# guisongchen/vo_slam_test

Measured on AMD Instinct MI355X. Metric: tracked frames/sec + local-BA LM-iters/sec (synthetic 640x480; value = tracked frames/sec: ORB extraction, frame post-processing, two guided searches with the culling / isInFrame steps between them and two pose-only solves per frame, one vo_tracker C call per batch), higher is better.
Workload: dtype u8; 1 GPU; tracked frame: ORB extract (640x480, 8-level pyramid, 1000 kpts) + undistort/depth/grid + searchByProjection vs last frame + solvePoseOnlySE3 + cullingOutliersBeforeLocalMap + isInFrame (refined pose) + searchByProjection vs local map + solvePoseOnlySE3; frames, depth and map resident in HBM; parallelism=frames sharded x1, no collective, batches_in_flight=2

## Files before the change

vo_slam_test_amd/csrc/orb.hip:

```cpp
#include "vo_common.h"

#include <cmath>
#include <mutex>
#include <vector>

namespace {

using namespace vo;

constexpr int kMaxLevels = 16;
constexpr int kEdge = 19;
constexpr int kBorder = kEdge - 3;
constexpr int kHalfPatch = 15;
constexpr int kTileP = 72;
constexpr int kFastCpw = 4;
constexpr int kMaxList = 1024;

__constant__ __attribute__((aligned(16))) uint32_t c_desc_tab[64][36];
const int8_t h_pattern[1024] = {
#include "orb_pattern.inc"
};

struct LevelGeom {
  int w, h, pitch;
// ... 346 lines not shown
        const lds_u8 *b = (const lds_u8 *)(uintptr_t)(unsigned)plist[i];
        pos = (int)(b - tile);
        const lds_u8 *c = b + sdelta + 2 * TP + 2;
        sc0 = c[TP + 1];
        const unsigned nb = max_u16(max_u16(max_u16(c[0], c[1]), max_u16(c[2], c[TP])),
                                    max_u16(max_u16(c[TP + 2], c[2 * TP]), max_u16(c[2 * TP + 1], c[2 * TP + 2])));
        keep = sc0 >= th && sc0 > (int)nb;
      }
      const unsigned long long mask = __builtin_amdgcn_ballot_w64(keep);
      const int off = kept + __builtin_amdgcn_mbcnt_hi((unsigned)(mask >> 32), __builtin_amdgcn_mbcnt_lo((unsigned)mask, 0u));
      if (keep && off < cap_cell) {
        const int y = pos / TP, x = pos - y * TP;
        slot[off] = (uint32_t)(x + 3 + xoff) | ((uint32_t)(y + 3 + yoff) << 12) | ((uint32_t)sc0 << 24);
      }
      kept += __popcll(mask);
    }
    return kept;
  };
  int running = 0;
  for (int round = 0; round < 2; round++) {
    const int th = round == 0 ? ini_th : min_th;
    const int np0 = walk(th, 0, ih);
    wave_sync();
    int np = np0;
    if (np <= list_cap - 64) {
      if (round == 1) {
        if (np > 64) np = refine_list(np, th, ring_k2);
        if (np > 64) np = refine_list(np, th, ring_k1);
        if (np > 64) np = refine_list(np, th, ring_k3);
      }
      score_list(np);
      wave_sync();
      running = nms_list(np, th, 0);
    } else {
      const int chunk_rows = max((list_cap - 64) / 64, 1) * ri;
      for (int r0 = 0; r0 < ih; r0 += chunk_rows) {
        const int n = walk(th, r0, min(r0 + chunk_rows, ih));
        wave_sync();
        score_list(n);
        wave_sync();
      }
      running = 0;
      for (int r0 = 0; r0 < ih; r0 += chunk_rows) {
        const int n = walk(th, r0, min(r0 + chunk_rows, ih));
        wave_sync();
        running = nms_list(n, th, running);
        wave_sync();
      }
    }
    if (running > 0) break;
    wave_sync();
  }
  if (lane == 0) *out_count = min(running, cap_cell);
}

template <int TP, bool BYTEWISE>
__attribute__((amdgpu_waves_per_eu(8, 8))) __global__ __launch_bounds__(256) void k_fast_cell(OrbDev P, FrameSrc src, uint32_t *cell_slots,
                                                   long long slots_frame_stride, int *cell_count,
                                                   int cells_per_frame, int tile_rows, int list_cap,
                                                   const int *__restrict__ cell_tab, int cell_begin, int cell_end) {
  extern __shared__ __attribute__((aligned(16))) uint8_t fast_lds[];
  const int lane = threadIdx.x & 63;
  const int wave = __builtin_amdgcn_readfirstlane((int)threadIdx.x >> 6);
  const int f = blockIdx.y;
  for (int cpw = 0; cpw < kFastCpw; cpw++) {
  const int cell = cell_begin + (blockIdx.x * 4 + wave) * kFastCpw + cpw;
  if (cell >= cell_end) return;
  if (cpw) wave_sync();
  const int tile_bytes = fast_align16(TP * tile_rows);
  lds_u8 *tile_raw = (lds_u8 *)fast_lds + wave * fast_cell_lds(TP, tile_rows, list_cap);
  lds_u16 *plist = (lds_u16 *)(tile_raw + 2 * tile_bytes);
  const int *cd = cell_tab + 16 * cell;
  const int l = cd[0], iniX = cd[1], iniY = cd[2], cw = cd[3], ch = cd[4], xoff = cd[5], yoff = cd[6];
  const int slot_off = cd[7], cap_cell = cd[8];
  int *out_count = cell_count + (long long)f * cells_per_frame + cell;
  const int iw = cw - 6, ih = ch - 6;
  if (iw <= 0 || ih <= 0) {
    if (lane == 0) *out_count = 0;
    continue;
  }
  int pitch;
  const uint8_t *img;
  if (l == 0) {
    pitch = src.img0_pitch;
    img = src.img0 + (long long)f * src.img0_frame_stride;
  } else {
    pitch = cd[9];
    img = src.pyr + (long long)f * src.pyr_frame_stride + (((long long)cd[11] << 32) | (unsigned)cd[10]);
  }
  const bool bytewise = BYTEWISE && l == 0;
  const int ox = bytewise ? 0 : (iniX & 3);
  lds_u8 *tile = tile_raw + ox;
  const uint8_t *g0 = img + (long long)iniY * pitch + (iniX - ox);
  if (!bytewise && TP == 48) {
    gmem_u8 *gb = (gmem_u8 *)g0;
#pragma unroll
    for (int k = 0; k < 3; k++) {
      const int idx = lane + 64 * k;
      const unsigned row = (unsigned)idx / 3u, chunk = (unsigned)idx - 3u * row;
      if (64 * k < 3 * ch && idx < 3 * ch)
        __builtin_amdgcn_global_load_lds(gb + (row * (unsigned)pitch + 16u * chunk), tile_raw + 1024 * k, 16, 0, 0);
    }
  } else if (!bytewise) {
    constexpr int LW = TP <= 64 ? 16 : 32, RG = 64 / LW, NB = 6;
    const int npr = (ox + cw + 3) >> 2;
    const int d = lane & (LW - 1), r = lane / LW;
    if (d < npr) {
      const unsigned goff = (unsigned)(r * pitch + 4 * d);
      lds_u8 *lt = tile_raw + r * TP + 4 * d;
      const int ng = (ch + RG - 1) / RG, last0 = max(ch - RG, 0);
      for (int gb = 0; gb < ng; gb += NB) {
        uint32_t v[NB];
        int row0[NB];
#pragma unroll
        for (int q = 0; q < NB; q++) {
          row0[q] = min(min(gb + q, ng - 1) * RG, last0);
          long long ro = (long long)row0[q] * pitch;
          asm("" : "+s"(ro));
          v[q] = *reinterpret_cast<const uint32_t *>(g0 + ro + goff);
        }
#pragma unroll
        for (int q = 0; q < NB; q++) {
          int lo = row0[q] * TP;
          asm("" : "+s"(lo));
          *(__attribute__((address_space(3))) uint32_t *)(lt + lo) = v[q];
        }
      }
    }
  } else {
    constexpr int NB = 8;
    for (int col = lane; col < cw; col += 64) {
      for (int rb = 0; rb < ch; rb += NB) {
        uint8_t v[NB];
        int row[NB];
#pragma unroll
        for (int q = 0; q < NB; q++) {
          row[q] = min(rb + q, ch - 1);
          v[q] = g0[(long long)row[q] * pitch + col];
        }
#pragma unroll
        for (int q = 0; q < NB; q++) tile_raw[row[q] * TP + col] = v[q];
      }
    }
  }
  for (int i = lane; i < tile_bytes / 16; i += 64)
    *(__attribute__((address_space(3))) u32x4_t *)(tile_raw + tile_bytes + 16 * i) = u32x4_t{0u, 0u, 0u, 0u};
  asm volatile("s_waitcnt vmcnt(0)" ::: "memory");
  wave_sync();
  fast_cell_body<TP>(tile, tile_bytes, plist, list_cap, iw, ih, P.ini_th, P.min_th,
                     cell_slots + (long long)f * slots_frame_stride + slot_off, cap_cell, xoff, yoff, out_count, lane);
  }
}

__device__ __forceinline__ int block_excl_scan(int v, int *wsum , int *total) {
  const int lane = threadIdx.x & 63, wave = threadIdx.x >> 6;
  int x = v;
#pragma unroll
  for (int o = 1; o < 64; o <<= 1) {
    int y = __shfl_up(x, o);
    if (lane >= o) x += y;
  }
  __syncthreads();
  if (lane == 63) wsum[wave] = x;
  __syncthreads();
  int base = 0, tot = 0;
  for (int w = 0; w < 4; w++) {
    if (w < wave) base += wsum[w];
    tot += wsum[w];
  }
  *total = tot;
  return base + x - v;
}

template <int CAP>
struct OctLds {
  unsigned short x0[2][CAP], y0[2][CAP], x1[2][CAP], y1[2][CAP];
  unsigned short cnt[2][CAP], seq[2][CAP];
  unsigned short prank[CAP];
  unsigned short order[CAP];
  unsigned short newpos_old[CAP];
  unsigned short newpos_child[CAP * 4];
  int ccount[CAP * 4];
  int cprefix[CAP];
  unsigned int best[CAP];
  int wsum[8];
  int s_m, s_cutoff, s_newsize, s_nexp, s_total;
};

__device__ __forceinline__ int quadrant_of(int kx, int ky, int x0, int y0, int x1, int y1) {
  const int midx = x0 + ((x1 - x0 + 1) >> 1);
  const int midy = y0 + ((y1 - y0 + 1) >> 1);
  return (kx < midx ? 0 : 1) + (ky < midy ? 0 : 2);
}

template <int CAP>
__attribute__((amdgpu_waves_per_eu(kOctWaves, kOctWaves))) __global__ __launch_bounds__(256) void k_octree(OrbDev P, const uint32_t *cell_slots,
                                                long long slots_frame_stride, const int *cell_count,
                                                int cells_per_frame, uint32_t *key_data,
                                                unsigned short *key_label, int keys_per_frame,
                                                int *cand_count, uint32_t *sel, int sel_per_frame,
                                                int *nk, int *err_flag) {
  __shared__ OctLds<CAP> S;
  const int tid = threadIdx.x;
  const int l = blockIdx.y, f = blockIdx.x;
  const LevelGeom &L = P.lv[l];
  uint32_t *kd = key_data + (long long)f * keys_per_frame + L.candBase;
  unsigned short *kl = key_label + (long long)f * keys_per_frame + L.candBase;
  const int *cc = cell_count + (long long)f * cells_per_frame + L.cellBase;
  const uint32_t *slots = cell_slots + (long long)f * slots_frame_stride + L.slotBase;
  const int N = L.quota;

  constexpr int KR = 8;
  uint32_t kreg[KR];
  int lreg[KR];
  int n = 0;
  bool inreg;
  if (L.nCells <= CAP * 4) {
    int *coff = S.ccount;
    for (int base = 0; base < L.nCells; base += 256) {
      const int c = base + tid;
      const int cnt = c < L.nCells ? cc[c] : 0;
      int tot;
      const int off = n + block_excl_scan(cnt, S.wsum, &tot);
      if (c < L.nCells) coff[c] = off;
      n += tot;
    }
    __syncthreads();
    const int ncand = min(n, L.candCap);
    inreg = ncand <= 256 * KR;
    auto slot_of = [&](int k) {
      int lo = 0, hi = L.nCells - 1;
      while (lo < hi) {
        const int mid = (lo + hi + 1) >> 1;
        if (coff[mid] <= k) lo = mid; else hi = mid - 1;
      }
      return (long long)lo * L.capCell + (k - coff[lo]);
    };
#pragma unroll
    for (int e = 0; e < KR; e++) {
      const int k = tid + 256 * e;
      kreg[e] = k < ncand ? slots[slot_of(k)] : 0u;
      lreg[e] = 0;
    }
#pragma unroll
    for (int e = 0; e < KR; e++) {
      const int k = tid + 256 * e;
      if (k < ncand) kd[k] = kreg[e];
    }
    for (int k = tid + 256 * KR; k < ncand; k += 256) kd[k] = slots[slot_of(k)];
  } else {
    for (int base = 0; base < L.nCells; base += 256) {
      const int c = base + tid;
      const int cnt = c < L.nCells ? cc[c] : 0;
      int tot;
      const int off = n + block_excl_scan(cnt, S.wsum, &tot);
      for (int e0 = 0; e0 < cnt; e0 += 4) {
        uint32_t v[4];
#pragma unroll
        for (int u = 0; u < 4; u++) v[u] = slots[(long long)c * L.capCell + min(e0 + u, cnt - 1)];
#pragma unroll
        for (int u = 0; u < 4; u++)
          if (e0 + u < cnt && off + e0 + u < L.candCap) kd[off + e0 + u] = v[u];
      }
      n += tot;
    }
    __syncthreads();
    __threadfence_block();
    inreg = min(n, L.candCap) <= 256 * KR;
#pragma unroll
    for (int e = 0; e < KR; e++) {
      const int k = tid + 256 * e;
      kreg[e] = (inreg && k < min(n, L.candCap)) ? kd[k] : 0u;
      lreg[e] = 0;
    }
  }
  if (n > L.candCap) {
    if (tid == 0) atomicExch(err_flag, 1);
    n = L.candCap;
  }
  if (tid == 0) cand_count[f * P.nlevels + l] = n;
  __syncthreads();
  __threadfence_block();
  auto for_keys = [&](auto body) {
    if (inreg) {
#pragma unroll
      for (int e = 0; e < KR; e++) {
        const int k = tid + 256 * e;
        if (k < n) body(k, kreg[e], lreg[e]);
      }
    } else {
      for (int k = tid; k < n; k += 256) {
        int lab = kl[k];
        const int lab0 = lab;
        body(k, kd[k], lab);
        if (lab != lab0) kl[k] = (unsigned short)lab;
      }
    }
  };

  int cur = 0;
  const int nIni = L.nIni;
  const int H = L.maxBY - kBorder;
  for (int i = tid; i < CAP * 4; i += 256) S.ccount[i] = 0;
  __syncthreads();
  if (!inreg)
    for (int k = tid; k < n; k += 256) kl[k] = 0xffff;
  for_keys([&](int, uint32_t kv, int &lab) {
    const int kx = kv & 0xfff;
    int b = (int)((float)kx / L.hX);
    b = min(max(b, 0), nIni - 1);
    lab = b;
    atomicAdd(&S.ccount[b], 1);
  });
  __syncthreads();
  int size = 0;
  {
    if (tid == 0) {
      int s = 0;
      for (int i = 0; i < nIni && s < CAP; i++) {
        const int c = S.ccount[i];
        S.newpos_old[i] = 0xffff;
        if (c == 0) continue;
        S.x0[0][s] = (unsigned short)(int)(L.hX * (float)i);
        S.x1[0][s] = (unsigned short)(int)(L.hX * (float)(i + 1));
        S.y0[0][s] = 0;
        S.y1[0][s] = (unsigned short)H;
        S.cnt[0][s] = (unsigned short)min(c, 65535);
        S.seq[0][s] = (unsigned short)s;
        S.newpos_old[i] = (unsigned short)s;
        s++;
      }
      S.s_newsize = s;
    }
    __syncthreads();
    size = S.s_newsize;
    for_keys([&](int, uint32_t, int &lab) { lab = S.newpos_old[lab]; });
    __syncthreads();
  }

  bool careful = false;
  bool finish = (n == 0);
  int guard = 0;
  while (!finish && guard++ < 64) {
    const int prevSize = size;
    int myflag[4], myrank[4];
    int local = 0;
    for (int e = 0; e < 4; e++) {
      const int pos = tid * 4 + e;
      myflag[e] = (pos < size && S.cnt[cur][pos] > 1) ? 1 : 0;
      local += myflag[e];
    }
    int m;
    int ex = block_excl_scan(local, S.wsum, &m);
    for (int e = 0; e < 4; e++) {
      const int pos = tid * 4 + e;
      myrank[e] = ex;
      ex += myflag[e];
      if (pos < CAP) S.prank[pos] = myflag[e] ? (unsigned short)myrank[e] : 0xffff;
      if (myflag[e]) S.order[myrank[e]] = (unsigned short)pos;
    }
    __syncthreads();
    if (careful && m > 1) {
      for (int j = tid; j < m; j += 256) {
        const int p2 = S.order[j];
        S.cprefix[j] = (int)(((unsigned int)S.cnt[cur][p2] << 16) | S.seq[cur][p2]);
      }
      __syncthreads();
      int mypos[CAP / 256], myr[CAP / 256];
#pragma unroll
      for (int u = 0; u < CAP / 256; u++) {
        const int j = tid + 256 * u;
        mypos[u] = -1, myr[u] = 0;
        if (j >= m) continue;
        mypos[u] = S.order[j];
        const unsigned int mykey = (unsigned int)S.cprefix[j];
        int r = 0;
        for (int i = 0; i < m; i++) r += ((unsigned int)S.cprefix[i] > mykey) ? 1 : 0;
        myr[u] = r;
      }
      __syncthreads();
#pragma unroll
      for (int u = 0; u < CAP / 256; u++)
        if (mypos[u] >= 0) {
          S.prank[mypos[u]] = (unsigned short)myr[u];
          S.order[myr[u]] = (unsigned short)mypos[u];
        }
      __syncthreads();
    }
    for (int i = tid; i < m * 4; i += 256) S.ccount[i] = 0;
    __syncthreads();
    for_keys([&](int, uint32_t kv, int &lab) {
      const int pos = lab;
      const int r = S.prank[pos];
      if (r == 0xffff) return;
      const int q = quadrant_of(kv & 0xfff, (kv >> 12) & 0xfff, S.x0[cur][pos], S.y0[cur][pos], S.x1[cur][pos],
                                S.y1[cur][pos]);
      atomicAdd(&S.ccount[r * 4 + q], 1);
    });
    __syncthreads();
    {
      int run_c = 0;
      int cutoff = m - 1;
      bool found = false;
      for (int base = 0; base < m; base += 256) {
        const int r = base + tid;
        int c = 0;
        if (r < m)
          for (int q = 0; q < 4; q++) c += S.ccount[r * 4 + q] > 0;
        int tot;
        const int exs = block_excl_scan(c, S.wsum, &tot);
        const int inc = run_c + exs + c;
        if (r < m) S.cprefix[r] = inc;
        run_c += tot;
      }
      __syncthreads();
      if (careful) {
        if (tid == 0) S.s_cutoff = m - 1;
        __syncthreads();
        for (int r = tid; r < m; r += 256) {
          const int sz = prevSize + S.cprefix[r] - (r + 1);
          if (sz >= N) atomicMin(&S.s_cutoff, r);
        }
        __syncthreads();
        cutoff = S.s_cutoff;
        found = true;
      }
      (void)found;
      const int totalChildren = m > 0 ? S.cprefix[cutoff] : 0;
      const int nxt = cur ^ 1;
      if (tid == 0) S.s_nexp = 0;
      __syncthreads();
      int nexp_local = 0;
      for (int r = tid; r <= cutoff && r < m; r += 256) {
        const int pos = S.order[r];
        const int base_r = totalChildren - S.cprefix[r];
        const int px0 = S.x0[cur][pos], py0 = S.y0[cur][pos], px1 = S.x1[cur][pos], py1 = S.y1[cur][pos];
        const int midx = px0 + ((px1 - px0 + 1) >> 1), midy = py0 + ((py1 - py0 + 1) >> 1);
        int after = 0;
        for (int q = 3; q >= 0; q--) {
          const int c = S.ccount[r * 4 + q];
          if (c == 0) {
            S.newpos_child[r * 4 + q] = 0xffff;
            continue;
          }
          const int np = base_r + after;
          after++;
          S.newpos_child[r * 4 + q] = (unsigned short)np;
          S.x0[nxt][np] = (unsigned short)((q & 1) ? midx : px0);
          S.x1[nxt][np] = (unsigned short)((q & 1) ? px1 : midx);
          S.y0[nxt][np] = (unsigned short)((q & 2) ? midy : py0);
          S.y1[nxt][np] = (unsigned short)((q & 2) ? py1 : midy);
          S.cnt[nxt][np] = (unsigned short)min(c, 65535);
          S.seq[nxt][np] = (unsigned short)(r * 4 + q);
          nexp_local += c > 1;
        }
      }
      if (nexp_local) atomicAdd(&S.s_nexp, nexp_local);
      int keptlocal = 0, kf[4];
      for (int e = 0; e < 4; e++) {
        const int pos = tid * 4 + e;
        const int r = pos < size ? S.prank[pos] : 0xffff;
        kf[e] = (pos < size && (r == 0xffff || r > cutoff)) ? 1 : 0;
        keptlocal += kf[e];
      }
      int keptTotal;
      int kex = block_excl_scan(keptlocal, S.wsum, &keptTotal);
      for (int e = 0; e < 4; e++) {
        const int pos = tid * 4 + e;
        if (!kf[e]) {
          if (pos < CAP) S.newpos_old[pos] = 0xffff;
          continue;
        }
        const int np = totalChildren + kex;
        kex++;
        S.newpos_old[pos] = (unsigned short)np;
        if (np < CAP) {
          S.x0[nxt][np] = S.x0[cur][pos];
          S.x1[nxt][np] = S.x1[cur][pos];
          S.y0[nxt][np] = S.y0[cur][pos];
          S.y1[nxt][np] = S.y1[cur][pos];
          S.cnt[nxt][np] = S.cnt[cur][pos];
          S.seq[nxt][np] = S.seq[cur][pos];
        }
      }
      __syncthreads();
      const int newsize = totalChildren + keptTotal;
      for_keys([&](int, uint32_t kv, int &lab) {
        const int pos = lab;
        const int r = S.prank[pos];
        if (r != 0xffff && r <= cutoff) {
          const int q = quadrant_of(kv & 0xfff, (kv >> 12) & 0xfff, S.x0[cur][pos], S.y0[cur][pos],
                                    S.x1[cur][pos], S.y1[cur][pos]);
          lab = S.newpos_child[r * 4 + q];
        } else {
          lab = S.newpos_old[pos];
        }
      });
      __syncthreads();
      const int nToExpand = S.s_nexp;
      cur = nxt;
      size = newsize;
      if (size > CAP - 4) {
        if (tid == 0) atomicExch(err_flag, 2);
        finish = true;
      }
      if (size >= N || size == prevSize)
        finish = true;
      else if (!careful && size + nToExpand * 3 > N)
        careful = true;
    }
    __syncthreads();
  }

  for (int i = tid; i < CAP; i += 256) S.best[i] = 0;
  __syncthreads();
  for_keys([&](int k, uint32_t kv, int &lab) {
    const int pos = lab;
    if (pos >= CAP) return;
    const unsigned int v = ((kv >> 24) << 16) | (unsigned int)(65535 - k);
    atomicMax(&S.best[pos], v);
  });
  __syncthreads();
  uint32_t *out = sel + (long long)f * sel_per_frame + L.selBase;
  const int nout = min(size, L.capSel);
  for (int i = tid; i < nout; i += 256) out[i] = kd[65535 - (S.best[i] & 0xffff)];
  if (tid == 0) nk[f * P.nlevels + l] = (n == 0) ? 0 : nout;
}

__device__ __forceinline__ int reflect101(int i, int n) {
  if (n == 1) return 0;
  while (i < 0 || i >= n) i = i < 0 ? -i : 2 * n - 2 - i;
  return i;
}
__device__ __forceinline__ int reflect101_near(int i, int n) { return i < 0 ? -i : (i >= n ? 2 * n - 2 - i : i); }

__global__ __launch_bounds__(256) void k_blur(OrbDev P, FrameSrc src, unsigned level_mask) {
  __shared__ uint8_t t[22][72];
  __shared__ int hs[22][64];
  const int kq[7] = {18, 34, 49, 55, 49, 34, 18};
  const int tid = threadIdx.x, f = blockIdx.y;
  int tile = blockIdx.x;
  int l = 0;
  while (l + 1 < P.nlevels && tile >= P.lv[l + 1].tileBase) l++;
  const LevelGeom &L = P.lv[l];
  if (!((level_mask >> l) & 1u)) return;
  tile -= L.tileBase;
  const int ty = tile / L.tilesX, tx = tile - ty * L.tilesX;
  const int x0 = tx * 64, y0 = ty * 16;
  int pitch;
  const uint8_t *img = level_plane(P, src, l, f, pitch);
  for (int idx = tid; idx < 22 * 70; idx += 256) {
    const int r = idx / 70, c = idx - r * 70;
    const int sy = reflect101(y0 + r - 3, L.h), sx = reflect101(x0 + c - 3, L.w);
    t[r][c] = img[(long long)sy * pitch + sx];
  }
  __syncthreads();
  for (int idx = tid; idx < 22 * 64; idx += 256) {
    const int r = idx >> 6, c = idx & 63;
    int acc = 0;
#pragma unroll
    for (int i = 0; i < 7; i++) acc += kq[i] * t[r][c + i];
    hs[r][c] = acc;
  }
  __syncthreads();
  uint8_t *dst = src.blur + (long long)f * src.blur_frame_stride + L.blur_off;
  for (int idx = tid; idx < 16 * 64; idx += 256) {
    const int r = idx >> 6, c = idx & 63;
    if (x0 + c >= L.w || y0 + r >= L.h) continue;
    int acc = 0;
#pragma unroll
    for (int j = 0; j < 7; j++) acc += kq[j] * hs[r + j][c];
    const int v = (acc + (1 << 15)) >> 16;
    dst[blur_tiled_off(x0 + c, y0 + r, L.pitch)] = (uint8_t)min(v, 255);
  }
}

constexpr int kBlurB = 16;
constexpr int kBlurF = 64 / kBlurB;
constexpr int kBlurMinW = 24, kBlurMinH = 4;
constexpr int kBlurRows = 36;

__global__ __launch_bounds__(256) void k_blur_groups(FrameSrc src, int lv0_generic, const int *__restrict__ job_tab,
                                                     int n_jobs, int n_frames) {
  const int lane = threadIdx.x & 63;
  const int job = blockIdx.x * 4 + __builtin_amdgcn_readfirstlane((int)threadIdx.x >> 6);
  if (job >= n_jobs) return;
  const int *sd = job_tab + 16 * job;
  const int l = sd[0], cb = sd[1], sy = sd[2], Lh = sd[3], Lpitch = sd[4], ngroups = sd[5], w = sd[11];
  if (l == 0 && lv0_generic) return;
  const int f0 = blockIdx.y * kBlurF, fo = lane / kBlurB;
  const bool fvalid = f0 + fo < n_frames;
  const int fl = fvalid ? fo : 0;
  const int G = min(cb * kBlurB + (lane & (kBlurB - 1)), ngroups - 1), x = 4 * G;
  int pitch;
  const uint8_t *img;
  unsigned fsrc;
  if (l == 0) {
    pitch = src.img0_pitch;
    img = src.img0 + (long long)f0 * src.img0_frame_stride;
    fsrc = (unsigned)(fl * src.img0_frame_stride);
  } else {
    pitch = sd[8];
    img = src.pyr + (long long)f0 * src.pyr_frame_stride + (((long long)sd[10] << 32) | (unsigned)sd[9]);
    fsrc = (unsigned)(fl * src.pyr_frame_stride);
  }
  const int Gu = cb * kBlurB + (lane & (kBlurB - 1));
  const bool tile_ok = fvalid && 4 * (Gu & ~3) < Lpitch && (Gu & ~3) < ngroups;
  uint8_t *dst = src.blur + (long long)f0 * src.blur_frame_stride + (((long long)sd[7] << 32) | (unsigned)sd[6]) +
                 (long long)fl * src.blur_frame_stride + (Gu >> 2) * 128;
  __shared__ __attribute__((aligned(16))) unsigned tr_all[4][4][64];
  unsigned (*tr)[64] = tr_all[threadIdx.x >> 6];
  const unsigned vC = fsrc + (unsigned)x, vL = vC - (G > 0 ? 4u : 0u), vR = vC + (x + 4 < pitch ? 4u : 0u);
  const bool edge_job = cb == 0 || (cb + 1) * kBlurB * 4 + 4 > w;
  unsigned selC = 0x07060504u, selRA = 0x07060504u, selRB = 0u, selL = 0x03020100u;
  bool caseB = false, left = false;
  if (edge_job) {
    auto srck = [&](int k) {
      int i = x - 4 + k;
      if (i > w - 1) i = 2 * (w - 1) - i;
      return min(max(i - (x - 4), 0), 11);
    };
    selC = 0, selRA = 0, selRB = 0;
#pragma unroll
    for (int b = 0; b < 4; b++) {
      const int kc = srck(4 + b), kr = srck(8 + b);
      selC |= (unsigned)min(kc, 7) << (8 * b);
      selRA |= (unsigned)min(max(kr - 4, 0), 7) << (8 * b);
      selRB |= (unsigned)min(kr, 7) << (8 * b);
    }
    caseB = x + 4 > w - 1;
    left = G == 0;
    selL = 0x01020304u;
  }
  const int y0 = sy * kBlurRows, y1 = min(Lh, y0 + kBlurRows);
  const unsigned K0 = 18u | (34u << 8) | (49u << 16) | (55u << 24);
  const unsigned K1 = 49u | (34u << 8) | (18u << 16);
  typedef unsigned short u16x2 __attribute__((ext_vector_type(2)));
  const u16x2 W01 = {18, 34}, W23 = {49, 55}, W45 = {49, 34};
  unsigned pr[7][4], prev[4] = {0u, 0u, 0u, 0u};
#pragma unroll
  for (int j = 0; j < 7; j++)
#pragma unroll
    for (int q = 0; q < 4; q++) pr[j][q] = 0;
  constexpr int RB = 7;
  for (int yb = y0 - 3; yb < y1 + 3; yb += RB) {
    unsigned Lr[RB], Cr[RB], Rr[RB];
#pragma unroll
    for (int u = 0; u < RB; u++) {
      const int yq = min(yb + u, y1 + 2);
      const uint8_t *row = img + (long long)reflect101_near(yq, Lh) * pitch;
      Lr[u] = *reinterpret_cast<const unsigned *>(row + vL);
      Cr[u] = *reinterpret_cast<const unsigned *>(row + vC);
      Rr[u] = *reinterpret_cast<const unsigned *>(row + vR);
    }
#pragma unroll
    for (int u = 0; u < RB; u++) {
      const int yy = yb + u;
      if (yy >= y1 + 3) break;
      unsigned Lw = Lr[u], Cw = Cr[u], Rw = Rr[u];
      if (edge_job) {
        const unsigned l2 = __builtin_amdgcn_perm(Rw, Cw, selL);
        const unsigned c2 = __builtin_amdgcn_perm(Cw, Lw, selC);
        const unsigned ra = __builtin_amdgcn_perm(Rw, Cw, selRA), rb = __builtin_amdgcn_perm(Cw, Lw, selRB);
        Lw = left ? l2 : Lw;
        Rw = caseB ? rb : ra;
        Cw = c2;
      }
      unsigned hn[4];
      hn[0] = __builtin_amdgcn_udot4(__builtin_amdgcn_alignbyte(Cw, Lw, 1), K0, __builtin_amdgcn_udot4(__builtin_amdgcn_alignbyte(Rw, Cw, 1), K1, 0u, false), false);
      hn[1] = __builtin_amdgcn_udot4(__builtin_amdgcn_alignbyte(Cw, Lw, 2), K0, __builtin_amdgcn_udot4(__builtin_amdgcn_alignbyte(Rw, Cw, 2), K1, 0u, false), false);
      hn[2] = __builtin_amdgcn_udot4(__builtin_amdgcn_alignbyte(Cw, Lw, 3), K0, __builtin_amdgcn_udot4(__builtin_amdgcn_alignbyte(Rw, Cw, 3), K1, 0u, false), false);
      hn[3] = __builtin_amdgcn_udot4(Cw, K0, __builtin_amdgcn_udot4(Rw, K1, 0u, false), false);
      unsigned outw = 0;
      unsigned a4[4];
#pragma unroll
      for (int q = 0; q < 4; q++) {
        pr[(u + 6) % 7][q] = prev[q] | (hn[q] << 16);
        prev[q] = hn[q];
        unsigned acc = (unsigned)__mul24(18, (int)hn[q]) + (1u << 15);
// ... 1812 lines not shown
```

Before: 341,200 frames/s.

## Restructure octree distribution kernel: packed LDS node state, DPP scans, fewer barriers

Reworks the per-level octree keypoint distribution kernel. Node rectangles and count/seq are packed into uint2/uint32 LDS arrays, and per-key labels are packed two to a register. Block scans now use DPP wave scans with double-buffered partial sums, which removes one barrier per scan. Several passes are fused: quadrant bits are cached in registers, child and kept-node remapping goes through a single newpos table, expandable counts ride in the high bits of the scan, and in the non-careful case the kept-node scan is skipped. The in-register and in-memory paths are split with a compile-time flag, and optional s_memtime timing stamps are added behind a macro. The aim is less LDS traffic, fewer barriers and less register pressure on a latency-bound kernel, at the cost of more intricate bit packing that could hide correctness bugs.

Result: no change. 342,800 frames/s, median of 6 (+0.5%).

```diff
diff --git a/vo_slam_test_amd/csrc/orb.hip b/vo_slam_test_amd/csrc/orb.hip
--- a/vo_slam_test_amd/csrc/orb.hip
+++ b/vo_slam_test_amd/csrc/orb.hip
@@ -522,46 +522,68 @@
   }
 }
 
-__device__ __forceinline__ int block_excl_scan(int v, int *wsum , int *total) {
+__device__ __forceinline__ int wave_incl_scan_i32(int x) {
+  x += __builtin_amdgcn_update_dpp(0, x, 0x111, 0xf, 0xf, false);
+  x += __builtin_amdgcn_update_dpp(0, x, 0x112, 0xf, 0xf, false);
+  x += __builtin_amdgcn_update_dpp(0, x, 0x114, 0xf, 0xf, false);
+  x += __builtin_amdgcn_update_dpp(0, x, 0x118, 0xf, 0xf, false);
+  x += __builtin_amdgcn_update_dpp(0, x, 0x142, 0xa, 0xf, false);
+  x += __builtin_amdgcn_update_dpp(0, x, 0x143, 0xc, 0xf, false);
+  return x;
+}
+__device__ __forceinline__ int block_excl_scan(int v, int *wsum , int &par, int *total) {
   const int lane = threadIdx.x & 63, wave = threadIdx.x >> 6;
-  int x = v;
-#pragma unroll
-  for (int o = 1; o < 64; o <<= 1) {
-    int y = __shfl_up(x, o);
-    if (lane >= o) x += y;
-  }
-  __syncthreads();
-  if (lane == 63) wsum[wave] = x;
+  const int x = wave_incl_scan_i32(v);
+  int *ws = wsum + 4 * par;
+  par ^= 1;
+  if (lane == 63) ws[wave] = x;
   __syncthreads();
   int base = 0, tot = 0;
+#pragma unroll
   for (int w = 0; w < 4; w++) {
-    if (w < wave) base += wsum[w];
-    tot += wsum[w];
-  }
-  *total = tot;
+    const int s = ws[w];
+    if (w < wave) base += s;
+    tot += s;
+  }
+  *total = __builtin_amdgcn_readfirstlane(tot);
   return base + x - v;
 }
 
 template <int CAP>
 struct OctLds {
-  unsigned short x0[2][CAP], y0[2][CAP], x1[2][CAP], y1[2][CAP];
-  unsigned short cnt[2][CAP], seq[2][CAP];
+  uint2 rect[2][CAP];
+  __attribute__((aligned(16))) unsigned int cs[2][CAP];
   unsigned short prank[CAP];
   unsigned short order[CAP];
   unsigned short newpos_old[CAP];
-  unsigned short newpos_child[CAP * 4];
-  int ccount[CAP * 4];
+  __attribute__((aligned(8))) unsigned short newpos[CAP * 4];
+  __attribute__((aligned(16))) int ccount[CAP * 4];
   int cprefix[CAP];
   unsigned int best[CAP];
   int wsum[8];
-  int s_m, s_cutoff, s_newsize, s_nexp, s_total;
+  int s_cutoff, s_newsize;
 };
 
-__device__ __forceinline__ int quadrant_of(int kx, int ky, int x0, int y0, int x1, int y1) {
+__device__ __forceinline__ int quadrant_of(uint32_t kv, uint2 rc) {
+  const int kx = kv & 0xfff, ky = (kv >> 12) & 0xfff;
+  const int x0 = rc.x & 0xffff, y0 = rc.x >> 16, x1 = rc.y & 0xffff, y1 = rc.y >> 16;
   const int midx = x0 + ((x1 - x0 + 1) >> 1);
   const int midy = y0 + ((y1 - y0 + 1) >> 1);
   return (kx < midx ? 0 : 1) + (ky < midy ? 0 : 2);
 }
+
+#ifdef VO_OCT_STAMPS
+constexpr int kOctStampSlots = 12;
+#define OCT_STAMP(slot)                                                             \
+  do {                                                                              \
+    unsigned long long t_;                                                          \
+    asm volatile("s_memtime %0\n s_waitcnt lgkmcnt(0)" : "=s"(t_)::"memory");       \
+    st_[slot] += (unsigned int)(t_ - tp_);                                          \
+    tp_ = t_;                                                                       \
+  } while (0)
+#else
+#define OCT_STAMP(slot) do {} while (0)
+#endif
 
 template <int CAP>
 __attribute__((amdgpu_waves_per_eu(kOctWaves, kOctWaves))) __global__ __launch_bounds__(256) void k_octree(OrbDev P, const uint32_t *cell_slots,
@@ -579,11 +601,21 @@
   const int *cc = cell_count + (long long)f * cells_per_frame + L.cellBase;
   const uint32_t *slots = cell_slots + (long long)f * slots_frame_stride + L.slotBase;
   const int N = L.quota;
+#ifdef VO_OCT_STAMPS
+  unsigned int st_[kOctStampSlots] = {};
+  unsigned long long tp_;
+  asm volatile("s_memtime %0\n s_waitcnt lgkmcnt(0)" : "=s"(tp_)::"memory");
+#endif
 
   constexpr int KR = 8;
   uint32_t kreg[KR];
-  int lreg[KR];
+  unsigned int lreg[KR / 2] = {};
+  auto lab_of = [&](int e) { return (int)((e & 1) ? lreg[e >> 1] >> 16 : lreg[e >> 1] & 0xffffu); };
+  auto set_lab = [&](int e, int v) {
+    lreg[e >> 1] = (e & 1) ? (lreg[e >> 1] & 0xffffu) | ((unsigned int)v << 16) : (lreg[e >> 1] & 0xffff0000u) | ((unsigned int)v & 0xffffu);
+  };
   int n = 0;
+  int par = 0;
   bool inreg;
   if (L.nCells <= CAP * 4) {
     int *coff = S.ccount;
@@ -591,7 +623,7 @@
       const int c = base + tid;
       const int cnt = c < L.nCells ? cc[c] : 0;
       int tot;
-      const int off = n + block_excl_scan(cnt, S.wsum, &tot);
+      const int off = n + block_excl_scan(cnt, S.wsum, par, &tot);
       if (c < L.nCells) coff[c] = off;
       n += tot;
     }
@@ -610,7 +642,6 @@
     for (int e = 0; e < KR; e++) {
       const int k = tid + 256 * e;
       kreg[e] = k < ncand ? slots[slot_of(k)] : 0u;
-      lreg[e] = 0;
     }
 #pragma unroll
     for (int e = 0; e < KR; e++) {
@@ -623,7 +654,7 @@
       const int c = base + tid;
       const int cnt = c < L.nCells ? cc[c] : 0;
       int tot;
-      const int off = n + block_excl_scan(cnt, S.wsum, &tot);
+      const int off = n + block_excl_scan(cnt, S.wsum, par, &tot);
       for (int e0 = 0; e0 < cnt; e0 += 4) {
         uint32_t v[4];
 #pragma unroll
@@ -641,7 +672,6 @@
     for (int e = 0; e < KR; e++) {
       const int k = tid + 256 * e;
       kreg[e] = (inreg && k < min(n, L.candCap)) ? kd[k] : 0u;
-      lreg[e] = 0;
     }
   }
   if (n > L.candCap) {
@@ -651,20 +681,28 @@
   if (tid == 0) cand_count[f * P.nlevels + l] = n;
   __syncthreads();
   __threadfence_block();
+  OCT_STAMP(0);
+  auto for_keys_mem = [&](auto body) {
+    for (int k = tid; k < n; k += 256) {
+      int lab = kl[k];
+      const int lab0 = lab;
+      body(k, kd[k], lab, -1);
+      if (lab != lab0) kl[k] = (unsigned short)lab;
+    }
+  };
   auto for_keys = [&](auto body) {
     if (inreg) {
 #pragma unroll
       for (int e = 0; e < KR; e++) {
         const int k = tid + 256 * e;
-        if (k < n) body(k, kreg[e], lreg[e]);
+        if (k < n) {
+          int lab = lab_of(e);
+          body(k, kreg[e], lab, e);
+          set_lab(e, lab);
+        }
       }
     } else {
-      for (int k = tid; k < n; k += 256) {
-        int lab = kl[k];
-        const int lab0 = lab;
-        body(k, kd[k], lab);
-        if (lab != lab0) kl[k] = (unsigned short)lab;
-      }
+      for_keys_mem(body);
     }
   };
 
@@ -672,10 +710,11 @@
   const int nIni = L.nIni;
   const int H = L.maxBY - kBorder;
   for (int i = tid; i < CAP * 4; i += 256) S.ccount[i] = 0;
+  for (int i = tid; i < CAP; i += 256) S.best[i] = 0;
   __syncthreads();
   if (!inreg)
     for (int k = tid; k < n; k += 256) kl[k] = 0xffff;
-  for_keys([&](int, uint32_t kv, int &lab) {
+  for_keys([&](int, uint32_t kv, int &lab, int) {
     const int kx = kv & 0xfff;
     int b = (int)((float)kx / L.hX);
     b = min(max(b, 0), nIni - 1);
@@ -689,53 +728,54 @@
       int s = 0;
       for (int i = 0; i < nIni && s < CAP; i++) {
         const int c = S.ccount[i];
+        S.ccount[i] = 0;
         S.newpos_old[i] = 0xffff;
         if (c == 0) continue;
-        S.x0[0][s] = (unsigned short)(int)(L.hX * (float)i);
-        S.x1[0][s] = (unsigned short)(int)(L.hX * (float)(i + 1));
-        S.y0[0][s] = 0;
-        S.y1[0][s] = (unsigned short)H;
-        S.cnt[0][s] = (unsigned short)min(c, 65535);
-        S.seq[0][s] = (unsigned short)s;
+        S.rect[0][s] = make_uint2((unsigned)(int)(L.hX * (float)i) & 0xffffu,
+                                  ((unsigned)(int)(L.hX * (float)(i + 1)) & 0xffffu) | ((unsigned)H << 16));
+        S.cs[0][s] = ((unsigned)min(c, 65535) << 16) | (unsigned)s;
         S.newpos_old[i] = (unsigned short)s;
         s++;
       }
       S.s_newsize = s;
     }
     __syncthreads();
-    size = S.s_newsize;
-    for_keys([&](int, uint32_t, int &lab) { lab = S.newpos_old[lab]; });
+    size = __builtin_amdgcn_readfirstlane(S.s_newsize);
+    for_keys([&](int, uint32_t, int &lab, int) { lab = S.newpos_old[lab]; });
     __syncthreads();
   }
-
+  OCT_STAMP(1);
+
+  auto run_passes = [&](auto inreg_c) {
+  constexpr bool INREG = decltype(inreg_c)::value;
   bool careful = false;
   bool finish = (n == 0);
   int guard = 0;
   while (!finish && guard++ < 64) {
     const int prevSize = size;
-    int myflag[4], myrank[4];
-    int local = 0;
-    for (int e = 0; e < 4; e++) {
+    unsigned int myexp = 0;
+    {
+      uint4 mycs = make_uint4(0, 0, 0, 0);
+      if (tid * 4 < CAP) mycs = reinterpret_cast<const uint4 *>(S.cs[cur])[tid];
+      const unsigned int mycs_e[4] = {mycs.x, mycs.y, mycs.z, mycs.w};
+      for (int e = 0; e < 4; e++) myexp |= (tid * 4 + e < size && (mycs_e[e] >> 16) > 1) ? 1u << e : 0u;
+    }
+    auto expandable = [&](int e) { return ((myexp >> e) & 1u) != 0; };
+    const int local = __builtin_popcount(myexp);
+    int m;
+    myexp |= (unsigned int)block_excl_scan(local, S.wsum, par, &m) << 16;
+    for (int e = 0, ex = (int)(myexp >> 16); e < 4; e++) {
       const int pos = tid * 4 + e;
-      myflag[e] = (pos < size && S.cnt[cur][pos] > 1) ? 1 : 0;
-      local += myflag[e];
-    }
-    int m;
-    int ex = block_excl_scan(local, S.wsum, &m);
-    for (int e = 0; e < 4; e++) {
-      const int pos = tid * 4 + e;
-      myrank[e] = ex;
-      ex += myflag[e];
-      if (pos < CAP) S.prank[pos] = myflag[e] ? (unsigned short)myrank[e] : 0xffff;
-      if (myflag[e]) S.order[myrank[e]] = (unsigned short)pos;
-    }
+      const bool fl = expandable(e);
+      if (pos < CAP) S.prank[pos] = fl ? (unsigned short)ex : 0xffff;
+      if (fl) S.order[ex] = (unsigned short)pos;
+      if (careful && fl) S.cprefix[ex] = (int)S.cs[cur][pos];
+      ex += fl ? 1 : 0;
+    }
+    if (tid == 0) S.s_cutoff = m - 1;
     __syncthreads();
+    OCT_STAMP(2);
     if (careful && m > 1) {
-      for (int j = tid; j < m; j += 256) {
-        const int p2 = S.order[j];
-        S.cprefix[j] = (int)(((unsigned int)S.cnt[cur][p2] << 16) | S.seq[cur][p2]);
-      }
-      __syncthreads();
       int mypos[CAP / 256], myr[CAP / 256];
 #pragma unroll
       for (int u = 0; u < CAP / 256; u++) {
@@ -757,117 +797,125 @@
         }
       __syncthreads();
     }
-    for (int i = tid; i < m * 4; i += 256) S.ccount[i] = 0;
+    OCT_STAMP(3);
+    unsigned int qbits = 0;
+    if constexpr (INREG) {
+      int slot[KR];
+#pragma unroll
+      for (int e = 0; e < KR; e++) {
+        const int pos = min(lab_of(e), CAP - 1);
+        const int r = S.prank[pos];
+        const int q = quadrant_of(kreg[e], S.rect[cur][pos]);
+        qbits |= (unsigned int)q << (2 * e);
+        slot[e] = (tid + 256 * e < n && r != 0xffff) ? r * 4 + q : -1;
+      }
+#pragma unroll
+      for (int e = 0; e < KR; e++)
+        if (slot[e] >= 0) atomicAdd(&S.ccount[slot[e]], 1);
+    } else {
+      for_keys_mem([&](int, uint32_t kv, int &lab, int) {
+        const int pos = lab;
+        const int r = S.prank[pos];
+        if (r == 0xffff) return;
+        atomicAdd(&S.ccount[r * 4 + quadrant_of(kv, S.rect[cur][pos])], 1);
+      });
+    }
     __syncthreads();
-    for_keys([&](int, uint32_t kv, int &lab) {
-      const int pos = lab;
-      const int r = S.prank[pos];
-      if (r == 0xffff) return;
-      const int q = quadrant_of(kv & 0xfff, (kv >> 12) & 0xfff, S.x0[cur][pos], S.y0[cur][pos], S.x1[cur][pos],
-                                S.y1[cur][pos]);
-      atomicAdd(&S.ccount[r * 4 + q], 1);
-    });
-    __syncthreads();
+    OCT_STAMP(4);
     {
       int run_c = 0;
-      int cutoff = m - 1;
-      bool found = false;
       for (int base = 0; base < m; base += 256) {
         const int r = base + tid;
         int c = 0;
-        if (r < m)
-          for (int q = 0; q < 4; q++) c += S.ccount[r * 4 + q] > 0;
+        if (r < m) {
+          const int4 cq4 = reinterpret_cast<const int4 *>(S.ccount)[r];
+          const int cq[4] = {cq4.x, cq4.y, cq4.z, cq4.w};
+          for (int q = 0; q < 4; q++) c += (cq[q] > 0 ? 1 : 0) + (cq[q] > 1 ? 0x10000 : 0);
+        }
         int tot;
-        const int exs = block_excl_scan(c, S.wsum, &tot);
+        const int exs = block_excl_scan(c, S.wsum, par, &tot);
         const int inc = run_c + exs + c;
-        if (r < m) S.cprefix[r] = inc;
+        if (r < m) {
+          S.cprefix[r] = inc;
+          if (careful && prevSize + (inc & 0xffff) - (r + 1) >= N) atomicMin(&S.s_cutoff, r);
+        }
         run_c += tot;
       }
-      __syncthreads();
+      int cutoff = m - 1, upto = run_c;
       if (careful) {
-        if (tid == 0) S.s_cutoff = m - 1;
         __syncthreads();
-        for (int r = tid; r < m; r += 256) {
-          const int sz = prevSize + S.cprefix[r] - (r + 1);
-          if (sz >= N) atomicMin(&S.s_cutoff, r);
-        }
-        __syncthreads();
-        cutoff = S.s_cutoff;
-        found = true;
-      }
-      (void)found;
-      const int totalChildren = m > 0 ? S.cprefix[cutoff] : 0;
+        cutoff = __builtin_amdgcn_readfirstlane(S.s_cutoff);
+        upto = m > 0 ? __builtin_amdgcn_readfirstlane(S.cprefix[cutoff]) : 0;
+      }
+      const int totalChildren = upto & 0xffff, nToExpand = upto >> 16;
+      OCT_STAMP(5);
       const int nxt = cur ^ 1;
-      if (tid == 0) S.s_nexp = 0;
-      __syncthreads();
-      int nexp_local = 0;
-      for (int r = tid; r <= cutoff && r < m; r += 256) {
+      for (int r = tid; r < m; r += 256) {
+        const int4 cq4 = reinterpret_cast<const int4 *>(S.ccount)[r];
+        reinterpret_cast<int4 *>(S.ccount)[r] = make_int4(0, 0, 0, 0);
+        const int cq[4] = {cq4.x, cq4.y, cq4.z, cq4.w};
+        if (r > cutoff) continue;
         const int pos = S.order[r];
-        const int base_r = totalChildren - S.cprefix[r];
-        const int px0 = S.x0[cur][pos], py0 = S.y0[cur][pos], px1 = S.x1[cur][pos], py1 = S.y1[cur][pos];
+        const int base_r = totalChildren - (S.cprefix[r] & 0xffff);
+        const uint2 rc = S.rect[cur][pos];
+        const int px0 = rc.x & 0xffff, py0 = rc.x >> 16, px1 = rc.y & 0xffff, py1 = rc.y >> 16;
         const int midx = px0 + ((px1 - px0 + 1) >> 1), midy = py0 + ((py1 - py0 + 1) >> 1);
         int after = 0;
+        unsigned int np01 = 0xffffffffu, np23 = 0xffffffffu;
+#pragma unroll
         for (int q = 3; q >= 0; q--) {
-          const int c = S.ccount[r * 4 + q];
-          if (c == 0) {
-            S.newpos_child[r * 4 + q] = 0xffff;
-            continue;
-          }
+          const int c = cq[q];
+          if (c == 0) continue;
           const int np = base_r + after;
           after++;
-          S.newpos_child[r * 4 + q] = (unsigned short)np;
-          S.x0[nxt][np] = (unsigned short)((q & 1) ? midx : px0);
-          S.x1[nxt][np] = (unsigned short)((q & 1) ? px1 : midx);
-          S.y0[nxt][np] = (unsigned short)((q & 2) ? midy : py0);
-          S.y1[nxt][np] = (unsigned short)((q & 2) ? py1 : midy);
-          S.cnt[nxt][np] = (unsigned short)min(c, 65535);
-          S.seq[nxt][np] = (unsigned short)(r * 4 + q);
-          nexp_local += c > 1;
+          unsigned int &half = q >= 2 ? np23 : np01;
+          half = (q & 1) ? (half & 0xffffu) | ((unsigned int)np << 16) : (half & 0xffff0000u) | ((unsigned int)np & 0xffffu);
+          if (np < CAP) {
+            S.rect[nxt][np] = make_uint2((unsigned)(((q & 1) ? midx : px0) & 0xffff) | ((unsigned)((q & 2) ? midy : py0) << 16),
+                                         (unsigned)(((q & 1) ? px1 : midx) & 0xffff) | ((unsigned)((q & 2) ? py1 : midy) << 16));
+            S.cs[nxt][np] = ((unsigned)min(c, 65535) << 16) | (unsigned)(r * 4 + q);
+          }
         }
-      }
-      if (nexp_local) atomicAdd(&S.s_nexp, nexp_local);
-      int keptlocal = 0, kf[4];
+        reinterpret_cast<uint2 *>(S.newpos)[pos] = make_uint2(np01, np23);
+      }
+      OCT_STAMP(6);
+      unsigned int kmask = 0;
+      int kbase, keptTotal;
+      if (!careful) {
+        for (int e = 0; e < 4; e++) kmask |= (tid * 4 + e < size && !expandable(e)) ? 1u << e : 0u;
+        kbase = totalChildren + tid * 4 - (int)(myexp >> 16);
+        keptTotal = size - m;
+      } else {
+        for (int e = 0; e < 4; e++) {
+          const int pos = tid * 4 + e;
+          const int r = pos < size ? S.prank[pos] : 0;
+          kmask |= (pos < size && (r == 0xffff || r > cutoff)) ? 1u << e : 0u;
+        }
+        kbase = totalChildren + block_excl_scan(__builtin_popcount(kmask), S.wsum, par, &keptTotal);
+      }
       for (int e = 0; e < 4; e++) {
+        if (!((kmask >> e) & 1u)) continue;
         const int pos = tid * 4 + e;
-        const int r = pos < size ? S.prank[pos] : 0xffff;
-        kf[e] = (pos < size && (r == 0xffff || r > cutoff)) ? 1 : 0;
-        keptlocal += kf[e];
-      }
-      int keptTotal;
-      int kex = block_excl_scan(keptlocal, S.wsum, &keptTotal);
-      for (int e = 0; e < 4; e++) {
-        const int pos = tid * 4 + e;
-        if (!kf[e]) {
-          if (pos < CAP) S.newpos_old[pos] = 0xffff;
-          continue;
+        const int np = kbase + __builtin_popcount(kmask & ((1u << e) - 1u));
+        const unsigned int np2 = ((unsigned int)np & 0xffffu) * 0x10001u;
+        reinterpret_cast<uint2 *>(S.newpos)[pos] = make_uint2(np2, np2);
+        if (np < CAP) {
+          S.rect[nxt][np] = S.rect[cur][pos];
+          S.cs[nxt][np] = S.cs[cur][pos];
         }
-        const int np = totalChildren + kex;
-        kex++;
-        S.newpos_old[pos] = (unsigned short)np;
-        if (np < CAP) {
-          S.x0[nxt][np] = S.x0[cur][pos];
-          S.x1[nxt][np] = S.x1[cur][pos];
-          S.y0[nxt][np] = S.y0[cur][pos];
-          S.y1[nxt][np] = S.y1[cur][pos];
-          S.cnt[nxt][np] = S.cnt[cur][pos];
-          S.seq[nxt][np] = S.seq[cur][pos];
-        }
       }
       __syncthreads();
+      OCT_STAMP(7);
       const int newsize = totalChildren + keptTotal;
-      for_keys([&](int, uint32_t kv, int &lab) {
-        const int pos = lab;
-        const int r = S.prank[pos];
-        if (r != 0xffff && r <= cutoff) {
-          const int q = quadrant_of(kv & 0xfff, (kv >> 12) & 0xfff, S.x0[cur][pos], S.y0[cur][pos],
-                                    S.x1[cur][pos], S.y1[cur][pos]);
-          lab = S.newpos_child[r * 4 + q];
-        } else {
-          lab = S.newpos_old[pos];
-        }
-      });
-      __syncthreads();
-      const int nToExpand = S.s_nexp;
+      if constexpr (INREG) {
+#pragma unroll
+        for (int e = 0; e < KR; e++) set_lab(e, S.newpos[min(lab_of(e), CAP - 1) * 4 + (int)((qbits >> (2 * e)) & 3u)]);
+      } else {
+        for_keys_mem([&](int, uint32_t kv, int &lab, int) {
+          const int pos = min(lab, CAP - 1);
+          lab = S.newpos[pos * 4 + quadrant_of(kv, S.rect[cur][pos])];
+        });
+      }
       cur = nxt;
       size = newsize;
       if (size > CAP - 4) {
@@ -880,21 +928,40 @@
         careful = true;
     }
     __syncthreads();
-  }
-
-  for (int i = tid; i < CAP; i += 256) S.best[i] = 0;
-  __syncthreads();
-  for_keys([&](int k, uint32_t kv, int &lab) {
+    OCT_STAMP(8);
+#ifdef VO_OCT_STAMPS
+    st_[10]++, st_[11] += careful ? 1 : 0;
+#endif
+  }
+  auto best_body = [&](int k, uint32_t kv, int &lab, int) {
     const int pos = lab;
     if (pos >= CAP) return;
     const unsigned int v = ((kv >> 24) << 16) | (unsigned int)(65535 - k);
     atomicMax(&S.best[pos], v);
-  });
+  };
+  if constexpr (INREG) {
+#pragma unroll
+    for (int e = 0; e < KR; e++) {
+      const int k = tid + 256 * e;
+      int lab = lab_of(e);
+      if (k < n) best_body(k, kreg[e], lab, e);
+    }
+  } else {
+    for_keys_mem(best_body);
+  }
+  };
+  if (inreg) run_passes(std::true_type{}); else run_passes(std::false_type{});
   __syncthreads();
   uint32_t *out = sel + (long long)f * sel_per_frame + L.selBase;
   const int nout = min(size, L.capSel);
   for (int i = tid; i < nout; i += 256) out[i] = kd[65535 - (S.best[i] & 0xffff)];
   if (tid == 0) nk[f * P.nlevels + l] = (n == 0) ? 0 : nout;
+#ifdef VO_OCT_STAMPS
+  __syncthreads();
+  OCT_STAMP(9);
+  if (tid == 0 && n >= kOctStampSlots)
+    for (int i = 0; i < kOctStampSlots; i++) kd[i] = st_[i];
+#endif
 }
 
 __device__ __forceinline__ int reflect101(int i, int n) {
```
